# astro-turing/Integrating-diagenetic-equations-using-Python

Hardware: AMD Instinct MI355X
Metric: grid-point-steps/sec (5 fields, fp64) (higher is better)
Workload: dtype f64

## Files before the change

integrating-diagenetic-equations-using-python_amd/csrc/marl_api.hip:

```cpp
#include <hip/hip_runtime.h>

#include <dlfcn.h>

#include <cmath>
#include <cstdarg>
#include <cstdio>
#include <cstring>
#include <string>
#include <vector>

#include "../../include/marl_hip.h"
#include "marl_kernels.h"
#include "marl_rk23_ctl.h"
#include "marl_rk4_watch_ctl.h"
#include "marl_radau.h"
#include "marl_radau_cr.h"
#include "marl_radau_batch.h"
#include "marl_radau_wg.h"
#include "marl_bdf.h"
#include "marl_bdf_wg.h"
#include "marl_bdf_batch.h"
#include "marl_devbuf.h"

using namespace marl;
// ... 19 lines not shown
    size_t part_cap = 0;
    unsigned* sq = nullptr;
    size_t sq_cap = 0;
    unsigned sq_item_base = 0, sq_level_base = 0;
    bool sq_test_raise = false;
    int64_t sq_max_items = 0x7fffffff;
    unsigned* sq_sticky = nullptr;
    unsigned* sq_host = nullptr;
    bool sq_pending = false;
    int cus = 0;
    Rk45Stream* rs = nullptr;
    double* rs_grec = nullptr;
    unsigned* rs_host = nullptr;
    unsigned rs_arrive_base = 0, rs_epoch_base = 0, rs_grab_base = 0, rs_G = 0, rs_grabs_per_attempt = 0;
    int rs_occ[3][2] = {{0, 0}, {0, 0}, {0, 0}};
    int64_t rk45_stream = 1;
    int64_t dd_stream = 0;
    int64_t rk45_stream_attempts = 4096;
    double* rec = nullptr;
    Rk45Ctrl* dctrl = nullptr;
    Rk45Ctrl* hctrl = nullptr;
    double* hrec = nullptr;
    double* ddt = nullptr;
    double* hdt = nullptr;
    double* sw_teval = nullptr;
    size_t sw_teval_cap = 0;
    int64_t* sw_ndone = nullptr;
    double* sw_tev = nullptr;
    size_t sw_tev_cap = 0;
    double* dop_k = nullptr;
    size_t dop_k_cap = 0;
    double* rk4w_recs = nullptr;
    size_t rk4w_recs_cap = 0;
    int64_t dop_grid_extra = -1;
    double* dd_send = nullptr;
    double* dd_gathered = nullptr;
    double* dd_recs = nullptr;
    int dd_rank = 0, dd_world = 1;
    int64_t dd_max_attempts = 0;
    void* rccl_lib = nullptr;
    void* rccl_comm = nullptr;
    int (*rccl_allgather)(const void*, void*, size_t, int, void*, hipStream_t) = nullptr;
    int (*rccl_destroy)(void*) = nullptr;
    double* rd_arena = nullptr;
    size_t rd_cap = 0;
    double* rd_host = nullptr;
    double* zc_h = nullptr;
    double* zc_d = nullptr;
    bool zc_on = false;
    int64_t rk4_variant = -1, sweep_variant = -1, host_layout = LAYOUT_TILED, poll = 64;
    int64_t rk4_stream = 1;
    int64_t rk4_small = 1;
    int64_t rk4_chain = 1;
    int64_t rk4_stream_third = 1;
    double* stream_c = nullptr;
    size_t stream_c_cap = 0;
    int64_t implicit_zero_copy = 1;
    int64_t radau_fused_solve = 3;
    int64_t radau_solver = 0;
    int64_t radau_cr = -1;
    int64_t radau_cr_min_n = 2048;
    int64_t radau_cr_small = 3;
    int64_t radau_cr_small_min_n = 205;
    int64_t bdf_solve_wg = 1;
    int64_t radau_cr_tail = 1;
    int64_t radau_sweep_wg = 3;
    int64_t terminal[7] = {0, 0, 0, 0, 0, 0, 0};
    std::string err;
};

static bool has_terminal(const marl_ctx* ctx)
{
    for (int e = 0; e < 7; e++)
        if (ctx->terminal[e] > 0) return true;
    return false;
}

static int fail(marl_ctx* ctx, int code, const char* fmt, ...);
#define NO_TERMINAL(ctx, entry) \
    if (has_terminal(ctx)) return fail(ctx, -1, "%s: terminal monitors are not supported by this entry (marl_set_terminal)", entry);

static int fail(marl_ctx* ctx, int code, const char* fmt, ...)
{
    char msg[512];
    va_list ap;
    va_start(ap, fmt);
    vsnprintf(msg, sizeof msg, fmt, ap);
    va_end(ap);
    if (ctx) ctx->err = msg; else g_create_error = msg;
    return code;
}

#define HIP_OK(ctx, call)                                                                         \
    do {                                                                                          \
        hipError_t e_ = (call);                                                                   \
        if (e_ != hipSuccess) return fail(ctx, -100 - (int)e_, "%s failed: %s", #call, hipGetErrorString(e_)); \
    } while (0)

#define LAUNCH_OK(ctx)                                                                            \
    do {                                                                                          \
        hipError_t e_ = hipGetLastError();                                                        \
        if (e_ != hipSuccess) return fail(ctx, -100 - (int)e_, "kernel launch failed: %s", hipGetErrorString(e_)); \
    } while (0)

#ifdef MARL_LAB_CLOCK45
extern "C" int marl_lab_read_clock45(unsigned long long* dst, size_t n)
// ... 227 lines not shown
        return fail(ctx, -2, "rk4: the streamed time loop gave up waiting for a neighbouring tile (rk4_stream_kernel); the state is invalid");
    }
    return 0;
}

int marl_set_terminal(marl_ctx* ctx, const int64_t terminal[7])
{
    if (!ctx) return -1;
    for (int e = 0; terminal && e < 7; e++)
        if (terminal[e] < 0) return fail(ctx, -1, "marl_set_terminal: limit %d is negative (0: never terminal; k > 0: stop at the k-th occurrence)", e);
    for (int e = 0; e < 7; e++) ctx->terminal[e] = terminal ? terminal[e] : 0;
    return 0;
}

int marl_synchronize(marl_ctx* ctx)
{
    if (!ctx) return -1;
    HIP_OK(ctx, hipStreamSynchronize(ctx->stream));
    return stream_check(ctx);
}

int marl_set_option(marl_ctx* ctx, const char* name, int64_t value)
{
    if (!ctx || !name) return -1;
    const std::string n(name);
    if (n == "rk4_variant") ctx->rk4_variant = value;
    else if (n == "rk45_variant") { }
    else if (n == "sweep_variant") ctx->sweep_variant = value;
    else if (n == "host_layout") ctx->host_layout = value ? LAYOUT_TILED : LAYOUT_FIELD_MAJOR;
    else if (n == "poll_interval") ctx->poll = value > 0 ? value : 1;
    else if (n == "radau_solver") {
#ifdef MARL_LAB_BLOCK_THOMAS
        ctx->radau_solver = value ? 1 : 0;
#else
        if (value) return fail(ctx, -1, "marl_set_option: radau_solver = 1 (sequential block Thomas, the cross-check of the cyclic-reduction solver) is compiled into lab builds only (-DMARL_LAB_BLOCK_THOMAS)");
        ctx->radau_solver = 0;
#endif
    }
    else if (n == "radau_cr") ctx->radau_cr = (value < 0) ? -1 : std::min<int64_t>(value, radau::CR_MAX_LEVELS);
    else if (n == "radau_cr_min_n") ctx->radau_cr_min_n = std::max<int64_t>(value, 4);
    else if (n == "radau_cr_small") ctx->radau_cr_small = value < 0 ? 0 : std::min<int64_t>(value, radau::CR_WG_MAX_LEVELS);
    else if (n == "radau_cr_small_min_n") ctx->radau_cr_small_min_n = std::max<int64_t>(value, 32);
    else if (n == "radau_cr_tail") ctx->radau_cr_tail = value ? 1 : 0;
    else if (n == "bdf_solve_wg") ctx->bdf_solve_wg = value ? 1 : 0;
    else if (n == "radau_fused_solve") ctx->radau_fused_solve = value < 0 ? 0 : (value > 3 ? 3 : value);
    else if (n == "radau_sweep_wg") ctx->radau_sweep_wg = value < 0 ? 0 : (value > 3 ? 3 : value);
    else if (n == "implicit_zero_copy") ctx->implicit_zero_copy = value ? 1 : 0;
    else if (n == "rk4_stream") ctx->rk4_stream = value < 0 ? 0 : (value > 2 ? 2 : value);
    else if (n == "rk45_stream") ctx->rk45_stream = value < 0 ? 0 : (value > 2 ? 2 : value);
    else if (n == "dd_stream") ctx->dd_stream = value < 0 ? 0 : (value > 2 ? 2 : value);
    else if (n == "rk45_stream_attempts") ctx->rk45_stream_attempts = value < 1 ? 1 : std::min<int64_t>(value, 1 << 20);
    else if (n == "rk4_small") ctx->rk4_small = value ? 1 : 0;
    else if (n == "rk4_chain") ctx->rk4_chain = value < 0 ? 0 : std::min<int64_t>(value, kChainMax);
    else if (n == "rk4_stream_third") ctx->rk4_stream_third = value ? 1 : 0;
    else if (n == "rk4_stream_test_raise") ctx->sq_test_raise = value != 0;
    else if (n == "rk4_stream_max_items") ctx->sq_max_items = value > 0 ? std::min<int64_t>(value, 0x7fffffff) : 0x7fffffff;
    else if (n == "no_reuse") {
        for (auto& c : ctx->hconsts) c.hot.no_reuse = value ? 1 : 0;
        HIP_OK(ctx, hipSetDevice(ctx->device));
        HIP_OK(ctx, hipStreamSynchronize(ctx->stream));
        HIP_OK(ctx, hipMemcpy(ctx->dconsts, ctx->hconsts.data(), sizeof(DevConsts) * ctx->hconsts.size(), hipMemcpyHostToDevice));
    }
    else return fail(ctx, -1, "marl_set_option: unknown option '%s'", name);
    return 0;
}

int marl_get_constants(const marl_ctx* ctx, int64_t inst, double out[19])
{
    if (!ctx || inst < 0 || inst >= ctx->batch || !out) return -1;
    const DevConsts& d = ctx->hconsts[inst];
    const HotConsts& c = d.hot;
    const double* x = &ctx->extra[4 * inst];
    const double v[19] = {x[0], c.nu1, c.nu2, c.KRat, c.dCa, c.dCO3, c.delta, c.Da, c.lambda_, x[1], x[2], c.rhorat,
                          c.presum, x[3], c.dPhi, PECLET_MIN, PECLET_MAX, (double)d.mask_lo, (double)d.mask_hi};
    memcpy(out, v, sizeof v);
    return 0;
}

int64_t marl_state_doubles(const marl_ctx* ctx, int layout) { return ctx ? state_doubles(ctx->slab.n_buf, layout) : -1; }

}

#ifndef MARL_LAB
static inline int64_t inst_stride(const marl_ctx* ctx, int layout) { return state_doubles(ctx->slab.n_buf, layout); }

static inline unsigned blocks256(int64_t n) { return (unsigned)((n + 255) / 256); }

static const ZBatch kNoBatch{0, nullptr, 0, 0, nullptr};

static int launch_rhs_fm(marl_ctx* ctx, const double* y, double* dydt, int64_t nstates, unsigned cnt = 1, const ZBatch& zb = kNoBatch,
                         int const_stride = 0)
{
    const dim3 grid(blocks256(ctx->slab.n_buf), (unsigned)nstates, cnt);
    const int64_t stride = inst_stride(ctx, LAYOUT_FIELD_MAJOR);
    if (ctx->var_dphi)
        hipLaunchKernelGGL((rhs_kernel<LAYOUT_FIELD_MAJOR, true>), grid, dim3(256), 0, ctx->stream, y, dydt, ctx->dconsts, ctx->slab, stride, const_stride, zb);
    else
        hipLaunchKernelGGL(rhs_kernel<LAYOUT_FIELD_MAJOR>, grid, dim3(256), 0, ctx->stream, y, dydt, ctx->dconsts, ctx->slab, stride, const_stride, zb);
    LAUNCH_OK(ctx);
    return 0;
}

static int launch_rhs(marl_ctx* ctx, const double* y, double* dydt, int layout, int64_t nstates = 0)
{
    if (layout != LAYOUT_TILED) return launch_rhs_fm(ctx, y, dydt, nstates > 0 ? nstates : ctx->batch, 1, kNoBatch, nstates > 0 ? 0 : 1);
    const dim3 grid(blocks256(ctx->slab.n_buf), (unsigned)(nstates > 0 ? nstates : ctx->batch));
// ... 99 lines not shown
    return 0;
}

static int default_rk4_depth(const marl_ctx* ctx)
{
    if (ctx->var_dphi) return kVdRk4Depth;
    if (ctx->rk4_variant >= 0 && ctx->rk4_variant < kNumRk4Depths) return kRk4Depths[ctx->rk4_variant];
    const int64_t n = ctx->slab.out_hi - ctx->slab.out_lo;
    return n <= 98304 ? 16 : (n <= 262144 ? 8 : 4);
}

#ifndef MARL_LAB_STREAM_BLK
#define MARL_LAB_STREAM_BLK 256
#endif
template <int NSTEPS, bool VD = false>
static void launch_stream_t(marl_ctx* ctx, double* a, double* b, int layout, double dt, unsigned levels, unsigned tiles, unsigned blocks, double* c = nullptr)
{
    if (layout == LAYOUT_TILED)
        hipLaunchKernelGGL((rk4_stream_kernel<MARL_LAB_STREAM_BLK, LAYOUT_TILED, NSTEPS, VD>), dim3(blocks), dim3(MARL_LAB_STREAM_BLK), 0, ctx->stream, a, b, ctx->dconsts, ctx->slab, dt,
                           levels, tiles, ctx->sq, ctx->sq + 2, ctx->sq_sticky, ctx->sq_item_base, ctx->sq_level_base, c);
    else
        hipLaunchKernelGGL((rk4_stream_kernel<MARL_LAB_STREAM_BLK, LAYOUT_FIELD_MAJOR, NSTEPS, VD>), dim3(blocks), dim3(MARL_LAB_STREAM_BLK), 0, ctx->stream, a, b, ctx->dconsts, ctx->slab,
                           dt, levels, tiles, ctx->sq, ctx->sq + 2, ctx->sq_sticky, ctx->sq_item_base, ctx->sq_level_base, c);
}

struct ChainShape {
    int64_t items, bound;
    unsigned K, nsub_last;
};
static ChainShape chain_shape(int64_t n, int64_t K)
{
    constexpr int64_t H = 16, V = 256 - 2 * H, W = 256 - H;
    static_assert(V % H == 0 && W % H == 0, "a clipped chain could be narrower than the halo");
    const int64_t bound = V * ((n - 1) / V), L = V + W * (K - 1);
    const int64_t chains = (bound + L - 1) / L;
    int64_t nsub_last = 0;
    if (chains > 0) {
        const int64_t R = bound - (chains - 1) * L;
        nsub_last = R <= V ? 1 : 1 + (R - V + W - 1) / W;
    }
    return {chains + 1, bound, (unsigned)K, (unsigned)nsub_last};
}

static int64_t rk4_chain_auto(int64_t n, int64_t resident)
{
    for (int64_t K = 8; K >= 2; K--)
        if (chain_shape(n, K).items >= 2 * resident) return K;
    return 1;
}

template <int LAYOUT>
static void launch_chain_t(marl_ctx* ctx, double* a, double* b, double dt, unsigned levels, const ChainShape& sh, unsigned blocks, double* c)
{
    hipLaunchKernelGGL((rk4_chain_kernel<256, LAYOUT, 4>), dim3(blocks), dim3(256), 0, ctx->stream, a, b, ctx->dconsts, ctx->slab, dt, levels,
                       (unsigned)sh.items, ctx->sq, ctx->sq + 2, ctx->sq_sticky, ctx->sq_item_base, ctx->sq_level_base, c, sh.K, sh.nsub_last, sh.bound);
}

static int rk4_stream(marl_ctx* ctx, double* a, double* b, int layout, double dt, int per, int64_t levels, double** result)
{
    const int64_t n = ctx->slab.out_hi - ctx->slab.out_lo, V = MARL_LAB_STREAM_BLK - 8 * per;
    if (!ctx->cus) {
        hipDeviceProp_t prop;
        HIP_OK(ctx, hipGetDeviceProperties(&prop, ctx->device));
        ctx->cus = prop.multiProcessorCount;
    }
    int64_t K = 1;
    if (per == 4 && !ctx->var_dphi && MARL_LAB_STREAM_BLK == 256 && ctx->rk4_chain > 0)
        K = ctx->rk4_chain == 1 ? rk4_chain_auto(n, 4 * (int64_t)ctx->cus) : ctx->rk4_chain;
    const ChainShape shape = chain_shape(n, K);
    const int64_t tiles = K >= 2 ? shape.items : (n + V - 1) / V;
    if (!ctx->sq_host) HIP_OK(ctx, hipHostMalloc((void**)&ctx->sq_host, sizeof(unsigned), hipHostMallocDefault));
    if (!ctx->sq_sticky) {
        HIP_OK(ctx, hipMalloc((void**)&ctx->sq_sticky, sizeof(unsigned)));
        HIP_OK(ctx, hipMemsetAsync(ctx->sq_sticky, 0, sizeof(unsigned), ctx->stream));
    }
    if (ctx->sq_cap < (size_t)tiles + 2 || ctx->sq_level_base > (1u << 30)) {
        if (ctx->sq_cap < (size_t)tiles + 2) {
            if (ctx->sq) HIP_OK(ctx, hipFree(ctx->sq));
            ctx->sq = nullptr;
            ctx->sq_cap = 0;
            HIP_OK(ctx, hipMalloc((void**)&ctx->sq, ((size_t)tiles + 2) * sizeof(unsigned)));
            ctx->sq_cap = (size_t)tiles + 2;
        }
        HIP_OK(ctx, hipMemsetAsync(ctx->sq, 0, ctx->sq_cap * sizeof(unsigned), ctx->stream));
        ctx->sq_item_base = ctx->sq_level_base = 0;
    }
    if (ctx->sq_test_raise) {
        HIP_OK(ctx, hipMemsetAsync(ctx->sq_sticky, 1, sizeof(unsigned), ctx->stream));
        ctx->sq_test_raise = false;
    }
    while (levels > 0) {
        const int64_t cap = (ctx->sq_max_items / tiles) & ~(int64_t)1;
        const int64_t lv = std::min<int64_t>(levels, std::max<int64_t>(cap, 2));
        const unsigned blocks = (unsigned)std::min<int64_t>(lv * tiles, (4 * 256 / MARL_LAB_STREAM_BLK) * (int64_t)ctx->cus);
        double* c = nullptr;
        if (ctx->rk4_stream_third && levels == lv && (lv & 1) && lv >= 3) {
            const size_t need = (size_t)state_doubles(ctx->slab.n_buf, layout);
            if (ctx->stream_c_cap < need) {
                if (ctx->stream_c) HIP_OK(ctx, hipFree(ctx->stream_c));
                ctx->stream_c = nullptr; ctx->stream_c_cap = 0;
                HIP_OK(ctx, hipMalloc((void**)&ctx->stream_c, need * sizeof(double)));
                ctx->stream_c_cap = need;
            }
            c = ctx->stream_c;
        }
        if (K >= 2) {
            if (layout == LAYOUT_TILED) launch_chain_t<LAYOUT_TILED>(ctx, a, b, dt, (unsigned)lv, shape, blocks, c);
            else launch_chain_t<LAYOUT_FIELD_MAJOR>(ctx, a, b, dt, (unsigned)lv, shape, blocks, c);
// ... 3147 lines not shown
```

integrating-diagenetic-equations-using-python_amd/csrc/marl_kernels.h:

```cpp
#pragma once
#include <type_traits>

#include "marl_math.h"
#include "marl_brent.h"
#include "marl_rk_ctrl.h"
#include "marl_rk_terminal.h"

namespace marl {

enum : int { LAYOUT_FIELD_MAJOR = 0, LAYOUT_TILED = 1 };

template <int LAYOUT>
__device__ __forceinline__ int64_t at(int f, int64_t i, int64_t ld)
{
    if constexpr (LAYOUT == LAYOUT_FIELD_MAJOR)
        return (int64_t)f * ld + i;
    else
        return (i >> 6) * (int64_t)(NF * 64) + f * 64 + (i & 63);
}

struct Slab {
    int64_t n_buf;
    int64_t goff;
    int64_t ld;
    int64_t out_lo;
    int64_t out_hi;
};

__device__ __forceinline__ double nanmin(double a, double b) { return (a < b || a != a) ? a : b; }
__device__ __forceinline__ double nanmax(double a, double b) { return (a > b || a != a) ? a : b; }
template <bool FINITE = false>
__device__ __forceinline__ double mon_min(double a, double b) { return FINITE ? __builtin_fmin(a, b) : nanmin(a, b); }
template <bool FINITE = false>
__device__ __forceinline__ double mon_max(double a, double b) { return FINITE ? __builtin_fmax(a, b) : nanmax(a, b); }


#ifdef MARL_LAB_PHASE_CLOCK
__device__ unsigned long long marl_lab_phase[8];
#define MARL_PHASE_MARK(k) do { const unsigned long long t_ = __builtin_amdgcn_s_memtime(); ph_acc[k] += t_ - ph_last; ph_last = t_; } while (0)
#else
#define MARL_PHASE_MARK(k) do { } while (0)
#endif

#define MARL_ONCE _Pragma("unroll") for (int once_ = 0; once_ < 1; once_++)
#define MARL_FIELDS _Pragma("unroll") for (int f = 0; f < NF; f++)

template <int BLK, bool REUSE = true, bool VD = false, int SEAM = 0>
struct StencilBlock {
    static constexpr int EDGE_DOUBLES = 2 * NF * BLK;
    static constexpr bool CACHE_LDS = PC_LDS_SLOTS > 0;
    static constexpr bool CACHE = REUSE && (EDGE_DOUBLES + TABLE_DOUBLES + PC_LDS_SLOTS * BLK) * 8 <= 60 * 1024;
    static constexpr int CACHE_DOUBLES = CACHE ? PC_LDS_SLOTS * BLK : 0;
    static constexpr int LDS_DOUBLES = EDGE_DOUBLES + TABLE_DOUBLES + CACHE_DOUBLES;

    double* lds;
    Tables T;
    HotConsts K;
    const DevConsts* C;
    int tid;
    int parity;
    unsigned masks;
    static constexpr bool EDGE_ONCE = CACHE;
    unsigned edge_cells;
    __device__ __forceinline__ bool edge_wave() const
    {
        if constexpr (SEAM > 0) {
            unsigned e = edge_cells;
            asm volatile("" : "+s"(e));
            return e & 1u;
        } else if constexpr (EDGE_ONCE) return edge_cells & 1u;
        else return __builtin_amdgcn_ballot_w64(is_edge() != 0) != 0;
    }
    bool w_zone = false;
    __device__ __forceinline__ unsigned edge_word() const { unsigned e = edge_cells; asm volatile("" : "+s"(e)); return e; }
    __device__ __forceinline__ unsigned is_first() const { if constexpr (SEAM > 0) return (unsigned)tid + 1u == ((edge_word() >> 8) & 0x1ffu); else return masks & 1u; }
    __device__ __forceinline__ unsigned is_last() const { if constexpr (SEAM > 0) return (unsigned)tid + 1u == ((edge_word() >> 20) & 0x1ffu); else return (masks >> 8) & 1u; }
    __device__ __forceinline__ unsigned in_zone() const { if constexpr (SEAM > 0) return w_zone; else return (masks >> 16) & 1u; }
    __device__ __forceinline__ unsigned is_edge() const { return masks & 0x101u; }
    PointCache<(CACHE && CACHE_LDS) ? BLK : 0> cache;
    bool reuse_live = false;
    static constexpr int SEAM_STRIDE = 16, SEAM_READS = 0x10000, SEAM_WAVE0 = 0x20000, SEAM_WAVEW = 0x40000;
    static_assert(SEAM < BLK, "the recording lane is a lane of the window");
    double* seam = nullptr;
    int seam_pos = 0;
#ifdef MARL_LAB_PHASE_CLOCK
    unsigned long long ph_acc[6] = {0, 0, 0, 0, 0, 0}, ph_last = __builtin_amdgcn_s_memtime();
    __device__ __forceinline__ void phase_flush()
    {
        if (threadIdx.x == 0)
            for (int k = 0; k < 6; k++) atomicAdd(&marl_lab_phase[k], ph_acc[k]);
    }
#endif

    __device__ __forceinline__ StencilBlock(double* lds_, int64_t g0, const DevConsts* __restrict__ c)
        : lds(lds_), T(load_tables(lds_ + EDGE_DOUBLES, BLK)), K(load_hot(c)), C(c), tid(threadIdx.x), parity(0)
    {
        if constexpr (SEAM > 0) set_interior(false);
        else set_window(g0);
        if constexpr (CACHE && CACHE_LDS) cache.s = lds_ + EDGE_DOUBLES + TABLE_DOUBLES + tid;
    }

    __device__ __forceinline__ void rebind(int t)
    {
        tid = t;
        if constexpr (CACHE && CACHE_LDS) cache.s = lds + EDGE_DOUBLES + TABLE_DOUBLES + t;
    }

    __device__ __forceinline__ void set_window(int64_t g)
    {
        const int64_t N = C->N, mlo = C->mask_lo, mhi = C->mask_hi;
        masks = ((g == 0) ? 1u : 0u) | ((g == N - 1) ? 0x100u : 0u) | ((g >= mlo && g < mhi) ? 0x10000u : 0u);
        edge_cells = 0;
        if constexpr (EDGE_ONCE) edge_cells = (__builtin_amdgcn_ballot_w64(is_edge() != 0) != 0) ? 1u : 0u;
    }

    __device__ __forceinline__ void set_window_seam(int64_t gw)
    {
        const int64_t N = C->N, mlo = C->mask_lo, mhi = C->mask_hi;
        const int64_t g = gw + tid;
        w_zone = g >= mlo && g < mhi;
        masks = 0;
        const int wave = __builtin_amdgcn_readfirstlane(tid) >> 6;
        const int64_t t0 = -gw, t1 = N - 1 - gw;
        unsigned e = 0;
        if (t0 >= 0 && t0 < BLK) e |= (((unsigned)t0 + 1u) << 8) | ((int)(t0 >> 6) == wave ? 1u : 0u);
        if (t1 >= 0 && t1 < BLK) e |= (((unsigned)t1 + 1u) << 20) | ((int)(t1 >> 6) == wave ? 1u : 0u);
        edge_cells = __builtin_amdgcn_readfirstlane(e);
    }

    __device__ __forceinline__ void set_interior(bool zone)
    {
        w_zone = zone;
        masks = 0;
        edge_cells = 0;
    }

    template <int MODE = TR_PLAIN>
    __device__ __forceinline__ void eval(const double (&ys)[NF], double (&k)[NF], PointAux& aux)
    {
        MARL_PHASE_MARK(4);
        double* e = lds + parity * (NF * BLK);
#pragma unroll
        for (int f = 0; f < NF; f++) e[f * BLK + tid] = ys[f];
        if constexpr (SEAM > 0) {
            if (seam_pos & SEAM_WAVEW) {
                int tw = tid;
                asm volatile("" : "+v"(tw));
                if (tw == SEAM) {
                    double* rec = seam + (seam_pos & 0xffff);
#pragma unroll
                    for (int f = 0; f < NF; f++) rec[f] = ys[f];
                }
            }
        }
        MARL_PHASE_MARK(0);
        PointLocal pl;
        MARL_ONCE point_local<CACHE ? MODE : TR_PLAIN, (CACHE && CACHE_LDS) ? BLK : 0, VD>(ys, in_zone(), K, C, T, pl, aux, cache, reuse_live);
        MARL_PHASE_MARK(1);
        __syncthreads();
        MARL_PHASE_MARK(2);
        const int tl = tid > 0 ? tid - 1 : 0;
        const int tr = tid < BLK - 1 ? tid + 1 : BLK - 1;
        double left[NF], right[NF];
#pragma unroll
        for (int f = 0; f < NF; f++) left[f] = e[f * BLK + tl];
        if constexpr (SEAM > 0) {
            if ((seam_pos & (SEAM_WAVE0 | SEAM_READS)) == (SEAM_WAVE0 | SEAM_READS)) {
                int t0 = tid;
                asm volatile("" : "+v"(t0));
                if (t0 == 0) {
                    const double* prev = seam + ((seam_pos & 0xffff) ^ 8);
#pragma unroll
                    for (int f = 0; f < NF; f++) left[f] = prev[f];
                }
            }
            seam_pos += SEAM_STRIDE;
        }
        const bool need_right_solids = __builtin_amdgcn_ballot_w64(!pl.upw) != 0;
        if constexpr (CACHE) {
#pragma unroll
            for (int f = 2; f < NF; f++) right[f] = e[f * BLK + tr];
            asm volatile("" : "=v"(right[0]), "=v"(right[1]));
            if (need_right_solids) {
                right[0] = e[tr];
                right[1] = e[BLK + tr];
            }
        } else {
#pragma unroll
            for (int f = 0; f < NF; f++) right[f] = (f >= 2 || need_right_solids) ? e[f * BLK + tr] : 0.0;
        }
        parity ^= 1;
        MARL_ONCE {
            double um[NF], up[NF];
#pragma unroll
            for (int f = 0; f < NF; f++) { um[f] = left[f]; up[f] = right[f]; }
            if (edge_wave()) {
                if (is_last()) {
#pragma unroll
                    for (int f = 0; f < NF; f++) up[f] = ghost_upper(f, ys[f], um[f]);
                }
                if constexpr (SEAM > 0) {
                    size_t off = offsetof(DevConsts, bc);
                    asm volatile("" : "+s"(off));
                    const double* bcp = reinterpret_cast<const double*>(reinterpret_cast<const char*>(C) + off);
                    double bcv[NF];
#pragma unroll
                    for (int f = 0; f < NF; f++) bcv[f] = bcp[f];
                    if (is_first()) {
#pragma unroll
                        for (int f = 0; f < NF; f++) um[f] = ghost_lower(bcv[f], ys[f]);
                    }
                } else if (is_first()) {
#pragma unroll
                    for (int f = 0; f < NF; f++) um[f] = ghost_lower(C->bc[f], ys[f]);
                }
            }
            point_rates<VD, true, !CACHE>(ys, um, up, K, T, pl, k, need_right_solids);
        }
#ifdef MARL_LAB_PHASE_CLOCK
        asm volatile("" :: "v"(k[0]), "v"(k[4]));
        MARL_PHASE_MARK(3);
        ph_acc[5]++;
#endif
    }
};

template <int BLK, int NQ, int NMIN, bool FINITE = false>
__device__ __forceinline__ void block_reduce(double (&q)[NQ], double* scratch)
{
    const int lane = threadIdx.x & 63, wave = threadIdx.x >> 6;
    constexpr int NW = BLK / 64;
    auto combine = [](int j, double a, double o) { return (j == 0) ? a + o : (j <= NMIN ? mon_min<FINITE>(a, o) : mon_max<FINITE>(a, o)); };
// ... 343 lines not shown
#pragma unroll
            for (int f = 0; f < NF; f++) __hip_atomic_store(dst + at<LAYOUT>(f, l, S.ld), y[f], __ATOMIC_RELAXED, __HIP_MEMORY_SCOPE_AGENT);
        }
        __atomic_signal_fence(__ATOMIC_SEQ_CST);
        __builtin_amdgcn_s_waitcnt(0);
        __atomic_signal_fence(__ATOMIC_SEQ_CST);
        __syncthreads();
        if (threadIdx.x == 0) {
            __hip_atomic_store(&done[tile], level_base + level + 1u, __ATOMIC_RELAXED, __HIP_MEMORY_SCOPE_AGENT);
#ifdef MARL_LAB_BROKEN_STREAM_LATCH
            s_item = __hip_atomic_fetch_add(&queue[0], 1u, __ATOMIC_RELAXED, __HIP_MEMORY_SCOPE_AGENT) - item_base;
            s_abort = 0;
#endif
        }
    }
}

struct ChainArgs {
    double *bufA, *bufB;
    const DevConsts* consts;
    Slab S;
    double dt;
    unsigned levels, items;
    unsigned *queue, *done, *sticky;
    unsigned item_base, level_base;
    double* bufC;
    unsigned K, nsub_last;
    int64_t bound;
};
static_assert(offsetof(ChainArgs, S) == 24 && offsetof(ChainArgs, dt) == 64 && offsetof(ChainArgs, queue) == 80 && offsetof(ChainArgs, bufC) == 112 &&
              offsetof(ChainArgs, bound) == 128 && sizeof(ChainArgs) == 136, "the argument list of rk4_chain_kernel, in order");
typedef const __attribute__((address_space(4))) ChainArgs* ChainArgsPtr;
__device__ __forceinline__ ChainArgsPtr chain_args()
{
    ChainArgsPtr a = (ChainArgsPtr)__builtin_amdgcn_kernarg_segment_ptr();
    asm volatile("" : "+s"(a));
    return a;
}

template <int BLK, int LAYOUT, int NSTEPS>
__global__ void __launch_bounds__(BLK) __attribute__((amdgpu_waves_per_eu(4, 8)))
rk4_chain_kernel(double* bufA, double* bufB, const DevConsts* __restrict__ consts, Slab S, double dt, unsigned levels, unsigned items,
                 unsigned* queue, unsigned* done, unsigned* sticky, unsigned item_base, unsigned level_base, double* bufC,
                 unsigned K, unsigned nsub_last, int64_t bound)
{
    constexpr int H = 4 * NSTEPS;
    constexpr int V = BLK - 2 * H;
    constexpr int W = BLK - H;
    static_assert(V > 0, "window too small for the fused halo");
    using SB = StencilBlock<BLK, true, false, BLK - H - 1>;
    __shared__ double lds[SB::LDS_DOUBLES];
    __shared__ double seam[H * SB::SEAM_STRIDE];
    __shared__ unsigned s_item, s_abort;
    const DevConsts& C = consts[0];
    SB sb(lds, 0, consts);
    sb.seam = seam;
    dt = pin_uniform(dt);
    const unsigned total = levels * items;
    const unsigned chains = items - 1;

    while (true) {
        __syncthreads();
        typedef __attribute__((address_space(1))) unsigned* GlobalWords;
        ChainArgsPtr G = chain_args();
        unsigned *const queue = (unsigned*)(GlobalWords)G->queue, *const done = (unsigned*)(GlobalWords)G->done,
                 *const sticky = (unsigned*)(GlobalWords)G->sticky;
        const unsigned items = G->items, item_base = G->item_base, level_base = G->level_base;
        if (threadIdx.x == 0) {
            s_item = __hip_atomic_fetch_add(&queue[0], 1u, __ATOMIC_RELAXED, __HIP_MEMORY_SCOPE_AGENT) - item_base;
            s_abort = 0;
        }
        __syncthreads();
        const unsigned item = __builtin_amdgcn_readfirstlane(s_item);
        if (item >= total) break;
        const unsigned level = item / items, tile = item - level * items;
        if (level > 0) {
            if (threadIdx.x < 3) {
                const int64_t t = (int64_t)tile - 1 + threadIdx.x;
                if (t >= 0 && t < (int64_t)items) {
                    unsigned spins = 0;
                    while ((int)(__hip_atomic_load(&done[t], __ATOMIC_RELAXED, __HIP_MEMORY_SCOPE_AGENT) - (level_base + level)) < 0) {
                        __builtin_amdgcn_s_sleep(4);
                        if (++spins > STREAM_SPIN_LIMIT ||
                            ((spins & 255u) == 0 && __hip_atomic_load(sticky, __ATOMIC_RELAXED, __HIP_MEMORY_SCOPE_AGENT))) {
                            __hip_atomic_store(sticky, 1u, __ATOMIC_RELAXED, __HIP_MEMORY_SCOPE_AGENT);
                            s_abort = 1;
                            break;
                        }
                    }
                }
            }
            __syncthreads();
            if (s_abort) break;
        }
        const double* src;
        double* dst;
        unsigned nsub;
        int64_t first, clip;
        {
            ChainArgsPtr A = chain_args();
            double *const pA = A->bufA, *const pB = A->bufB, *const pC = A->bufC;
            const unsigned nlev = A->levels, KK = A->K, nlast = A->nsub_last;
            const int64_t olo = A->S.out_lo, ohi = A->S.out_hi, bnd = A->bound;
            src = (const double*)(const __attribute__((address_space(1))) double*)(pC ? (level == 0 ? pA : ((level & 1u) ? pB : pC)) : ((level & 1u) ? pB : pA));
            dst = (double*)(__attribute__((address_space(1))) double*)(pC ? (level + 1 == nlev ? pA : ((level & 1u) ? pC : pB)) : ((level & 1u) ? pA : pB));
            const bool chain = tile < chains;
// ... 1539 lines not shown
```

integrating-diagenetic-equations-using-python_amd/csrc/marl_math.h:

```cpp
#pragma once
#include <hip/hip_runtime.h>
#include <stddef.h>
#include <stdint.h>

#include "marl_tables.h"

namespace marl {

constexpr int NF = 5;

struct HotConsts {
    double inv_dx, inv_dx2;
    double presum, rhorat;
    double KRat, nu1, nu2;
    double lambda_, Da, delta;
    double dCa, dCO3, dPhi;
    double pe_cCa, pe_cCO3, pe_Phi;
    double m1, m2, n1, n2;
    double hdx;
    double pe_smax;
    double Dal;
    double Da_nu1, Dal_nu2;
    double rr10;
    double dPhi_dx2;
// ... 98 lines not shown
__device__ __forceinline__ double pow_sat(double b, double e, const Tables& T)
{
    const double r = fast_exp(e * fast_log(b, T), T);
    return (b == 0.0) ? 0.0 : r;
}

template <bool SERIES>
__device__ __forceinline__ double fv_sigma(double Pe, double W, const Tables& T)
{
    const double a = fabs(Pe);
    double s = 0.0;
    if (a > PECLET_MAX) {
        s = (W > 0.0) ? 1.0 : ((W < 0.0) ? -1.0 : W);
    } else if (!(a < PECLET_MIN)) {
        if (SERIES && a <= FV_SERIES_MAX) {
            const double x2 = Pe * Pe;
            double p = 2.3106432599002624e-11;
            p = __builtin_fma(p, x2, -2.2805151204592183e-10);
            p = __builtin_fma(p, x2, 2.2507846516808994e-09);
            p = __builtin_fma(p, x2, -2.2214608789979678e-08);
            p = __builtin_fma(p, x2, 2.1925947851873778e-07);
            p = __builtin_fma(p, x2, -2.1644042808063972e-06);
            p = __builtin_fma(p, x2, 2.1377799155576935e-05);
            p = __builtin_fma(p, x2, -1.0 / 4725);
            p = __builtin_fma(p, x2, 2.0 / 945);
            p = __builtin_fma(p, x2, -1.0 / 45);
            p = __builtin_fma(p, x2, 1.0 / 3);
            s = p * Pe;
        } else {
            s = (1.0 + 2.0 * rcp_nr(fast_exp(2.0 * Pe, T) - 1.0)) - rcp_nr(Pe);
        }
    }
    return s;
}

__device__ __forceinline__ double ghost_lower(double bc, double u0) { return 2.0 * bc - u0; }
__device__ __forceinline__ double ghost_upper(int f, double uN1, double uN2) { return (f < 2) ? 2.0 * uN1 - uN2 : uN1; }

struct PointAux {
    double U, W;
};

enum : int { TR_PLAIN = 0, TR_FILL = 1, TR_REUSE = 2, TR_AUTO = 3 };
constexpr double REUSE_LIMIT = 5e-5;
constexpr double REUSE_TINY = 2e-6;

#ifndef MARL_CACHE_LDS_SLOTS
#define MARL_CACHE_LDS_SLOTS 4
#endif
enum : int { PC_INVPHI, PC_INVOM, PC_INVDEN, PC_IB, PC_E, PC_TC, PC_SLOTS };
constexpr int PC_FIRST_LDS = PC_SLOTS - (MARL_CACHE_LDS_SLOTS < PC_SLOTS ? MARL_CACHE_LDS_SLOTS : PC_SLOTS);
constexpr int PC_LDS_SLOTS = PC_SLOTS - PC_FIRST_LDS;

template <int STRIDE>
struct PointCache {
    static constexpr int FIRST_LDS = STRIDE > 0 ? PC_FIRST_LDS : PC_SLOTS;
    double Phi, O2, cPhi, nib;
    double* s;
    double v[FIRST_LDS > 0 ? FIRST_LDS : 1];
    bool fv_quiet;
    __device__ __forceinline__ double get(int j) const { return j < FIRST_LDS ? v[j] : s[(j - FIRST_LDS) * STRIDE]; }
    __device__ __forceinline__ void set(int j, double x) { if (j < FIRST_LDS) v[j] = x; else s[(j - FIRST_LDS) * STRIDE] = x; }
};

template <int MODE>
__device__ __forceinline__ double ten_operand()
{
    if constexpr (MODE == TR_PLAIN) return 10.0;
    else return pin_uniform(10.0);
}

struct PointLocal {
    double Ux, R0, R1;
    double W, invPhi, G2, G3;
    double h1x, h2f;
    double Q4, DaR;
    double Wd;
    bool upw, fv_active;
    bool fv_solutes;
};

#pragma clang diagnostic push
#pragma clang diagnostic ignored "-Wsometimes-uninitialized"
template <int MODE, int STRIDE, bool VD = false, bool LEGACY = false>
__device__ __forceinline__ void point_local(const double (&uc)[NF], bool in_mask, const HotConsts& K, const DevConsts* __restrict__ C,
                                            const Tables& T, PointLocal& pl, PointAux& aux, PointCache<STRIDE>& pc, bool& live)
{
    static_assert(!LEGACY || MODE == TR_PLAIN, "the legacy operation order is the stand-alone RHS's (no transcendental cache)");
#ifdef MARL_ABLATE_CORE
    aux.U = aux.W = 0.0;
    return;
#endif
    const double CA = uc[0], CC = uc[1], c = uc[2], o = uc[3], Phi = uc[4];
    const double omPhi = 1.0 - Phi;
    const double O2 = c * o;

    double den, invPhi, invom, invden, ex, tC, tA;
    bool fv_check = K.fv != 0;
    bool reuse = false;
    if constexpr (MODE == TR_FILL) live = false;
    if ((MODE == TR_REUSE || MODE == TR_AUTO) && live) {
        const double d = Phi - pc.Phi, dO = O2 - pc.O2;
        const double v = dO * pc.nib;
        const double big = __builtin_fma(fabs(d), pc.cPhi, fabs(v));
        reuse = __builtin_amdgcn_ballot_w64(!(big < REUSE_LIMIT)) == 0;
        live = reuse;
        if (reuse) {
            const bool tiny = __builtin_amdgcn_ballot_w64(!(big < REUSE_TINY)) == 0;
            const double invPhi0 = pc.get(PC_INVPHI), invom0 = pc.get(PC_INVOM), invden0 = pc.get(PC_INVDEN), ib0 = pc.get(PC_IB);
            const double e0 = pc.get(PC_E), tC0 = pc.get(PC_TC);
            const double x = d * invPhi0, y = d * invom0, u = dO * ib0;
            double l1p, ip, w, gy;
            double da;
            if (__builtin_expect(tiny, 1)) {
                l1p = x * __builtin_fma(x, -0.5, 1.0);
                const double t10 = invPhi0 * __builtin_fma(-x, x, x);
                ip = invPhi0 - t10;
                da = 10.0 * t10;
                w = v * __builtin_fma(u, -0.5, 1.0);
                gy = __builtin_fma(y, 1.0 + y, 1.0);
            } else {
                l1p = x * __builtin_fma(x, __builtin_fma(x, 1.0 / 3, -0.5), 1.0);
                ip = invPhi0 * __builtin_fma(-x, __builtin_fma(-x, 1.0 - x, 1.0), 1.0);
                da = -10.0 * (ip - invPhi0);
                w = v * __builtin_fma(u, __builtin_fma(u, 1.0 / 3, -0.5), 1.0);
                gy = __builtin_fma(y, __builtin_fma(y, 1.0 + y, 1.0), 1.0);
            }
            const double z = -2.0 * l1p * invden0;
            invPhi = ip;
            invom = invom0 * gy;
            if (__builtin_expect(tiny, 1)) {
                invden = __builtin_fma(-invden0, __builtin_fma(-z, z, z), invden0);
                ex = e0 * __builtin_fma(da, __builtin_fma(da, 0.5, 1.0), 1.0);
                tC = tC0 * __builtin_fma(w, __builtin_fma(w, 0.5, 1.0), 1.0);
            } else {
                invden = invden0 * __builtin_fma(-z, __builtin_fma(-z, 1.0 - z, 1.0), 1.0);
                ex = e0 * __builtin_fma(da, __builtin_fma(da, __builtin_fma(da, 1.0 / 6, 0.5), 1.0), 1.0);
                tC = tC0 * __builtin_fma(w, __builtin_fma(w, __builtin_fma(w, 1.0 / 6, 0.5), 1.0), 1.0);
            }
            fv_check = !pc.fv_quiet;
            if (fv_check) {
                asm volatile("");
                den = rcp_nr(invden);
            }
        }
    }
    if (!reuse) {
#ifdef MARL_ABLATE_LOG
        const double L = Phi - 1.0;
#else
        const double L = fast_log(Phi, T);
#endif
        den = __builtin_fma(-2.0, L, 1.0);
        const double pd = Phi * den, od = omPhi * den, po = Phi * omPhi;
#ifdef MARL_ABLATE_RCP
        const double rall = 2.0 - pd * omPhi;
#else
        const double rall = rcp_nr(pd * omPhi);
#endif
        invPhi = rall * od, invom = rall * pd, invden = rall * po;
#ifdef MARL_ABLATE_EXP
        ex = 0.01 * __builtin_fma(-10.0, invPhi, 10.0);
#else
        const double ten = ten_operand<MODE>();
        ex = fast_exp(__builtin_fma(-ten, invPhi, ten), T);
#endif
        const bool over = O2 > 1.0;
        const double nsel = over ? K.n1 : K.n2;
#ifdef MARL_ABLATE_POW
        const double pwC = fabs(O2 - 1.0) * nsel;
#else
        const double pwC = pow_sat(fabs(O2 - 1.0), nsel, T);
#endif
        tC = (LEGACY ? (over ? 1.0 : -K.nu2) : (over ? K.Dal : -K.Dal_nu2)) * pwC;
        if (K.generic_p0) {
            asm volatile("");
            const double y1 = C->p0_n1, y2 = C->p0_n2, nu2 = C->hot.nu2;
            const double pcw = (O2 == 1.0) ? (over ? y1 : y2) : pwC;
            tC = (LEGACY ? 1.0 : K.Dal) * (over ? pcw - nu2 * y2 : y1 - nu2 * pcw);
        }
        if constexpr (MODE == TR_FILL || MODE == TR_AUTO) {
            const double ib = (K.generic_p0 | K.no_reuse) ? __builtin_nan("") : rcp_nr(O2 - 1.0);
            pc.Phi = Phi; pc.O2 = O2; pc.nib = nsel * ib;
            pc.cPhi = fmax(fmax(fabs(invPhi), fabs(invom)), fmax(12.0 * (invPhi * invPhi), 2.2 * fabs(invPhi * invden)));
            pc.set(PC_INVPHI, invPhi); pc.set(PC_INVOM, invom); pc.set(PC_INVDEN, invden); pc.set(PC_E, ex);
            pc.set(PC_IB, ib); pc.set(PC_TC, tC);
            live = true;
        }
    }
    {
        const double O3 = O2 * K.KRat;
        const bool under = O3 < 1.0;
        tA = O3 - O3;
        if (!under || in_mask) {
#ifdef MARL_ABLATE_POWA
            const double pwA = fabs(O3 - 1.0) * (under ? K.m2 : K.m1);
#else
            const double pwA = pow_sat(fabs(O3 - 1.0), under ? K.m2 : K.m1, T);
#endif
            tA = (LEGACY ? (under ? 1.0 : -K.nu1) : (under ? K.Da : -K.Da_nu1)) * pwA;
        }
        if (K.generic_p0) {
            asm volatile("");
            const double z1 = C->p0_m1, z2 = C->p0_m2, nu1 = C->hot.nu1;
            const double mask = in_mask ? 1.0 : 0.0;
            const double pa = (O3 == 1.0) ? (under ? z2 : z1) : ((!under || in_mask) ? fast_exp((under ? K.m2 : K.m1) * fast_log(fabs(O3 - 1.0), T), T) : 0.0);
            tA = (LEGACY ? 1.0 : K.Da) * (under ? pa * mask - nu1 * z1 : z2 * mask - nu1 * pa);
        }
    }
    const double rF = LEGACY ? K.rhorat * (1.0 - ex) : __builtin_fma(-K.rhorat, ex, K.rhorat);
    const double t2 = rF * (Phi * Phi);
    const double W = K.presum - t2;
    const double U = __builtin_fma(t2 * Phi, invom, K.presum);
    aux.U = U;
    aux.W = W;
    double wpe = fabs(W) * K.pe_Phi;
    if constexpr (VD) {
        const double dPhi = K.auxcon * ((1.0 - ex) * (Phi * Phi)) * (Phi * invom);
        wpe = fabs(W) * (K.pe_Phi * (K.dPhi * rcp_nr(dPhi)));
    }

    const double DA = LEGACY ? K.Da * (CA * tA) : CA * tA;
    const double DC = LEGACY ? K.Dal * (CC * tC) : CC * tC;
    const double DmD = DA - DC;
    const double DaR = omPhi * DmD;
    pl.upw = U > 0.0;
    pl.Ux = fabs(U * K.inv_dx);
    pl.R0 = __builtin_fma(CA, DmD, -DA);
    pl.R1 = __builtin_fma(CC, DmD, DC);

    bool fv_active = false;
    if constexpr (MODE == TR_PLAIN) pl.Wd = 0.0;
#ifdef MARL_ABLATE_FV
    fv_check = false;
#endif
    pl.fv_solutes = MODE != TR_PLAIN;
    if (fv_check) {
        asm volatile("");
        const double Wd = W * den;
// ... 111 lines not shown
```

Measured before the change: 53.66 billion.

## Add RK4 exchange kernel with cell-major LDS stencil and paired cache slots

Adds an rk4_exchange_kernel variant of the chained RK4 streaming kernel, selected by default through a new rk4_exchange option. It stores the neighbour-exchange stencil in LDS cell-major with a padded pitch, so each point's fields are written and read with 16-byte vector accesses. It also packs the transcendental cache slots in pairs so they move as double2 loads and stores. The aim is fewer LDS instructions per stencil evaluation. The kernel also asserts an LDS budget that allows four workgroups per CU. The cost is padding and possible bank conflicts from the strided cell layout.

Result: faster. 54.51 billion (median of 6 runs) (+1.6%).

```diff
diff --git a/integrating-diagenetic-equations-using-python_amd/csrc/marl_api.hip b/integrating-diagenetic-equations-using-python_amd/csrc/marl_api.hip
--- a/integrating-diagenetic-equations-using-python_amd/csrc/marl_api.hip
+++ b/integrating-diagenetic-equations-using-python_amd/csrc/marl_api.hip
@@ -95,6 +95,7 @@
     int64_t rk4_stream = 1;
     int64_t rk4_small = 1;
     int64_t rk4_chain = 1;
+    int64_t rk4_exchange = 1;
     int64_t rk4_stream_third = 1;
     double* stream_c = nullptr;
     size_t stream_c_cap = 0;
@@ -428,6 +429,11 @@
     else if (n == "rk45_stream_attempts") ctx->rk45_stream_attempts = value < 1 ? 1 : std::min<int64_t>(value, 1 << 20);
     else if (n == "rk4_small") ctx->rk4_small = value ? 1 : 0;
     else if (n == "rk4_chain") ctx->rk4_chain = value < 0 ? 0 : std::min<int64_t>(value, kChainMax);
+#ifdef MARL_LAB_XCH_PARTS
+    else if (n == "rk4_exchange") ctx->rk4_exchange = value < 0 ? 0 : std::min<int64_t>(value, 3);
+#else
+    else if (n == "rk4_exchange") ctx->rk4_exchange = value ? 1 : 0;
+#endif
     else if (n == "rk4_stream_third") ctx->rk4_stream_third = value ? 1 : 0;
     else if (n == "rk4_stream_test_raise") ctx->sq_test_raise = value != 0;
     else if (n == "rk4_stream_max_items") ctx->sq_max_items = value > 0 ? std::min<int64_t>(value, 0x7fffffff) : 0x7fffffff;
@@ -633,8 +639,18 @@
 template <int LAYOUT>
 static void launch_chain_t(marl_ctx* ctx, double* a, double* b, double dt, unsigned levels, const ChainShape& sh, unsigned blocks, double* c)
 {
-    hipLaunchKernelGGL((rk4_chain_kernel<256, LAYOUT, 4>), dim3(blocks), dim3(256), 0, ctx->stream, a, b, ctx->dconsts, ctx->slab, dt, levels,
-                       (unsigned)sh.items, ctx->sq, ctx->sq + 2, ctx->sq_sticky, ctx->sq_item_base, ctx->sq_level_base, c, sh.K, sh.nsub_last, sh.bound);
+#define MARL_CHAIN_LAUNCH(KERNEL)                                                                                                                \
+    hipLaunchKernelGGL(KERNEL, dim3(blocks), dim3(256), 0, ctx->stream, a, b, ctx->dconsts, ctx->slab, dt, levels, (unsigned)sh.items, ctx->sq, \
+                       ctx->sq + 2, ctx->sq_sticky, ctx->sq_item_base, ctx->sq_level_base, c, sh.K, sh.nsub_last, sh.bound)
+    switch (ctx->rk4_exchange) {
+        case 0: MARL_CHAIN_LAUNCH((rk4_chain_kernel<256, LAYOUT, 4>)); break;
+#ifdef MARL_LAB_XCH_PARTS
+        case 1: MARL_CHAIN_LAUNCH((rk4_exchange_kernel<256, LAYOUT, 4, XCH_CELL>)); break;
+        case 2: MARL_CHAIN_LAUNCH((rk4_exchange_kernel<256, LAYOUT, 4, XCH_PAIRS>)); break;
+#endif
+        default: MARL_CHAIN_LAUNCH((rk4_exchange_kernel<256, LAYOUT, 4>)); break;
+    }
+#undef MARL_CHAIN_LAUNCH
 }
 
 static int rk4_stream(marl_ctx* ctx, double* a, double* b, int layout, double dt, int per, int64_t levels, double** result)
diff --git a/integrating-diagenetic-equations-using-python_amd/csrc/marl_kernels.h b/integrating-diagenetic-equations-using-python_amd/csrc/marl_kernels.h
--- a/integrating-diagenetic-equations-using-python_amd/csrc/marl_kernels.h
+++ b/integrating-diagenetic-equations-using-python_amd/csrc/marl_kernels.h
@@ -45,9 +45,12 @@
 #define MARL_ONCE _Pragma("unroll") for (int once_ = 0; once_ < 1; once_++)
 #define MARL_FIELDS _Pragma("unroll") for (int f = 0; f < NF; f++)
 
-template <int BLK, bool REUSE = true, bool VD = false, int SEAM = 0>
+enum : int { XCH_CELL = 1, XCH_PAIRS = 2 };
+template <int BLK, bool REUSE = true, bool VD = false, int SEAM = 0, int XCH = 0>
 struct StencilBlock {
-    static constexpr int EDGE_DOUBLES = 2 * NF * BLK;
+    static constexpr bool CELL = (XCH & XCH_CELL) != 0, PAIRS = (XCH & XCH_PAIRS) != 0;
+    static constexpr int PITCH = NF + 1;
+    static constexpr int EDGE_DOUBLES = 2 * (CELL ? PITCH : NF) * BLK;
     static constexpr bool CACHE_LDS = PC_LDS_SLOTS > 0;
     static constexpr bool CACHE = REUSE && (EDGE_DOUBLES + TABLE_DOUBLES + PC_LDS_SLOTS * BLK) * 8 <= 60 * 1024;
     static constexpr int CACHE_DOUBLES = CACHE ? PC_LDS_SLOTS * BLK : 0;
@@ -77,7 +80,9 @@
     __device__ __forceinline__ unsigned is_last() const { if constexpr (SEAM > 0) return (unsigned)tid + 1u == ((edge_word() >> 20) & 0x1ffu); else return (masks >> 8) & 1u; }
     __device__ __forceinline__ unsigned in_zone() const { if constexpr (SEAM > 0) return w_zone; else return (masks >> 16) & 1u; }
     __device__ __forceinline__ unsigned is_edge() const { return masks & 0x101u; }
-    PointCache<(CACHE && CACHE_LDS) ? BLK : 0> cache;
+    static_assert(XCH == 0 || (CACHE && PC_LDS_SLOTS == 4 && (EDGE_DOUBLES + TABLE_DOUBLES) % 2 == 0), "XCH: 16-byte accesses, two pairs of cache slots");
+    PointCache<(CACHE && CACHE_LDS) ? BLK : 0, PAIRS> cache;
+    __device__ __forceinline__ double* cache_slots(double* l, int t) const { return l + EDGE_DOUBLES + TABLE_DOUBLES + (PAIRS ? 2 * t : t); }
     bool reuse_live = false;
     static constexpr int SEAM_STRIDE = 16, SEAM_READS = 0x10000, SEAM_WAVE0 = 0x20000, SEAM_WAVEW = 0x40000;
     static_assert(SEAM < BLK, "the recording lane is a lane of the window");
@@ -97,13 +102,13 @@
     {
         if constexpr (SEAM > 0) set_interior(false);
         else set_window(g0);
-        if constexpr (CACHE && CACHE_LDS) cache.s = lds_ + EDGE_DOUBLES + TABLE_DOUBLES + tid;
+        if constexpr (CACHE && CACHE_LDS) cache.s = cache_slots(lds_, tid);
     }
 
     __device__ __forceinline__ void rebind(int t)
     {
         tid = t;
-        if constexpr (CACHE && CACHE_LDS) cache.s = lds + EDGE_DOUBLES + TABLE_DOUBLES + t;
+        if constexpr (CACHE && CACHE_LDS) cache.s = cache_slots(lds, t);
     }
 
     __device__ __forceinline__ void set_window(int64_t g)
@@ -139,9 +144,16 @@
     __device__ __forceinline__ void eval(const double (&ys)[NF], double (&k)[NF], PointAux& aux)
     {
         MARL_PHASE_MARK(4);
-        double* e = lds + parity * (NF * BLK);
-#pragma unroll
-        for (int f = 0; f < NF; f++) e[f * BLK + tid] = ys[f];
+        double* e = lds + parity * ((CELL ? PITCH : NF) * BLK);
+        if constexpr (CELL) {
+            double* own = e + PITCH * tid;
+            reinterpret_cast<double2v*>(own)[0] = double2v{ys[0], ys[1]};
+            reinterpret_cast<double2v*>(own)[1] = double2v{ys[2], ys[3]};
+            own[4] = ys[4];
+        } else {
+#pragma unroll
+            for (int f = 0; f < NF; f++) e[f * BLK + tid] = ys[f];
+        }
         if constexpr (SEAM > 0) {
             if (seam_pos & SEAM_WAVEW) {
                 int tw = tid;
@@ -162,8 +174,15 @@
         const int tl = tid > 0 ? tid - 1 : 0;
         const int tr = tid < BLK - 1 ? tid + 1 : BLK - 1;
         double left[NF], right[NF];
-#pragma unroll
-        for (int f = 0; f < NF; f++) left[f] = e[f * BLK + tl];
+        if constexpr (CELL) {
+            const double* lc = e + PITCH * tl;
+            const double2v s01 = reinterpret_cast<const double2v*>(lc)[0], s23 = reinterpret_cast<const double2v*>(lc)[1];
+            left[0] = s01.x; left[1] = s01.y; left[2] = s23.x; left[3] = s23.y;
+            left[4] = lc[4];
+        } else {
+#pragma unroll
+            for (int f = 0; f < NF; f++) left[f] = e[f * BLK + tl];
+        }
         if constexpr (SEAM > 0) {
             if ((seam_pos & (SEAM_WAVE0 | SEAM_READS)) == (SEAM_WAVE0 | SEAM_READS)) {
                 int t0 = tid;
@@ -177,7 +196,17 @@
             seam_pos += SEAM_STRIDE;
         }
         const bool need_right_solids = __builtin_amdgcn_ballot_w64(!pl.upw) != 0;
-        if constexpr (CACHE) {
+        if constexpr (CELL) {
+            const double* rc = e + PITCH * tr;
+            const double2v s23 = reinterpret_cast<const double2v*>(rc)[1];
+            right[2] = s23.x; right[3] = s23.y;
+            right[4] = rc[4];
+            asm volatile("" : "=v"(right[0]), "=v"(right[1]));
+            if (need_right_solids) {
+                const double2v s01 = reinterpret_cast<const double2v*>(rc)[0];
+                right[0] = s01.x; right[1] = s01.y;
+            }
+        } else if constexpr (CACHE) {
 #pragma unroll
             for (int f = 2; f < NF; f++) right[f] = e[f * BLK + tr];
             asm volatile("" : "=v"(right[0]), "=v"(right[1]));
@@ -627,6 +656,144 @@
     __shared__ double lds[SB::LDS_DOUBLES];
     __shared__ double seam[H * SB::SEAM_STRIDE];
     __shared__ unsigned s_item, s_abort;
+    const DevConsts& C = consts[0];
+    SB sb(lds, 0, consts);
+    sb.seam = seam;
+    dt = pin_uniform(dt);
+    const unsigned total = levels * items;
+    const unsigned chains = items - 1;
+
+    while (true) {
+        __syncthreads();
+        typedef __attribute__((address_space(1))) unsigned* GlobalWords;
+        ChainArgsPtr G = chain_args();
+        unsigned *const queue = (unsigned*)(GlobalWords)G->queue, *const done = (unsigned*)(GlobalWords)G->done,
+                 *const sticky = (unsigned*)(GlobalWords)G->sticky;
+        const unsigned items = G->items, item_base = G->item_base, level_base = G->level_base;
+        if (threadIdx.x == 0) {
+            s_item = __hip_atomic_fetch_add(&queue[0], 1u, __ATOMIC_RELAXED, __HIP_MEMORY_SCOPE_AGENT) - item_base;
+            s_abort = 0;
+        }
+        __syncthreads();
+        const unsigned item = __builtin_amdgcn_readfirstlane(s_item);
+        if (item >= total) break;
+        const unsigned level = item / items, tile = item - level * items;
+        if (level > 0) {
+            if (threadIdx.x < 3) {
+                const int64_t t = (int64_t)tile - 1 + threadIdx.x;
+                if (t >= 0 && t < (int64_t)items) {
+                    unsigned spins = 0;
+                    while ((int)(__hip_atomic_load(&done[t], __ATOMIC_RELAXED, __HIP_MEMORY_SCOPE_AGENT) - (level_base + level)) < 0) {
+                        __builtin_amdgcn_s_sleep(4);
+                        if (++spins > STREAM_SPIN_LIMIT ||
+                            ((spins & 255u) == 0 && __hip_atomic_load(sticky, __ATOMIC_RELAXED, __HIP_MEMORY_SCOPE_AGENT))) {
+                            __hip_atomic_store(sticky, 1u, __ATOMIC_RELAXED, __HIP_MEMORY_SCOPE_AGENT);
+                            s_abort = 1;
+                            break;
+                        }
+                    }
+                }
+            }
+            __syncthreads();
+            if (s_abort) break;
+        }
+        const double* src;
+        double* dst;
+        unsigned nsub;
+        int64_t first, clip;
+        {
+            ChainArgsPtr A = chain_args();
+            double *const pA = A->bufA, *const pB = A->bufB, *const pC = A->bufC;
+            const unsigned nlev = A->levels, KK = A->K, nlast = A->nsub_last;
+            const int64_t olo = A->S.out_lo, ohi = A->S.out_hi, bnd = A->bound;
+            src = (const double*)(const __attribute__((address_space(1))) double*)(pC ? (level == 0 ? pA : ((level & 1u) ? pB : pC)) : ((level & 1u) ? pB : pA));
+            dst = (double*)(__attribute__((address_space(1))) double*)(pC ? (level + 1 == nlev ? pA : ((level & 1u) ? pC : pB)) : ((level & 1u) ? pA : pB));
+            const bool chain = tile < chains;
+            nsub = chain ? (tile + 1 == chains ? nlast : KK) : 1u;
+            first = olo - H + (chain ? (int64_t)tile * (V + (int64_t)W * (KK - 1)) : bnd);
+            clip = chain ? olo + bnd : ohi;
+        }
+#pragma unroll 1
+        for (unsigned j = 0; j < nsub; j++) {
+            int tid = threadIdx.x;
+            asm volatile("" : "+v"(tid));
+            sb.rebind(tid);
+            ChainArgsPtr A = chain_args();
+            const int64_t n_buf = A->S.n_buf, goff = A->S.goff, ld = A->S.ld;
+            const int64_t lw = first + (int64_t)j * W, gw = lw + goff;
+            const int64_t mlo = C.mask_lo, mhi = C.mask_hi;
+            auto neg = [](int64_t a, int64_t b) {
+                int32_t hi = (int32_t)(((uint64_t)a - (uint64_t)b) >> 32);
+                asm("" : "+s"(hi));
+                return hi;
+            };
+            const int32_t out_any = neg(lw, 0) | neg(n_buf, lw + BLK) | neg(gw, 1) | neg(C.N - 1, gw + BLK);
+            const int32_t zone_part = neg(gw, mlo) | neg(mhi, gw + BLK);
+            const int32_t zone_some = neg(mlo, gw + BLK) & neg(gw, mhi);
+            const bool interior = out_any >= 0 && (zone_part >= 0 || zone_some >= 0);
+            const int64_t l = lw + tid;
+            bool in = true;
+            int64_t la = l;
+            if (!interior) {
+                asm volatile("");
+                in = l >= 0 && l < n_buf;
+                la = in ? l : 0;
+            }
+            double y[NF];
+#pragma unroll
+            for (int f = 0; f < NF; f++) y[f] = __hip_atomic_load(src + at<LAYOUT>(f, la, ld), __ATOMIC_RELAXED, __HIP_MEMORY_SCOPE_AGENT);
+            if (interior) {
+                sb.set_interior(zone_part >= 0);
+            } else {
+                asm volatile("");
+#pragma unroll
+                for (int f = 0; f < NF; f++) y[f] = in ? y[f] : C.bc[f];
+                sb.set_window_seam(gw);
+            }
+            sb.reuse_live = false;
+            const int wave = __builtin_amdgcn_readfirstlane(tid) >> 6;
+            sb.seam_pos = (int)(j & 1u) * 8 + (j ? SB::SEAM_READS : 0) + (wave == 0 ? SB::SEAM_WAVE0 : 0)
+                          + (wave == (BLK - H - 1) / 64 ? SB::SEAM_WAVEW : 0);
+            const int64_t room = clip - lw;
+            int hi = neg(room, BLK - H) < 0 ? (int)room : BLK - H;
+            asm volatile("" : "+s"(hi));
+            rk4_advance<NSTEPS>(sb, y, dt);
+            int sp = sb.seam_pos;
+            asm volatile("" : "+s"(sp));
+            const int lo = (sp & SB::SEAM_READS) ? 0 : H;
+            int ts = threadIdx.x;
+            asm volatile("" : "+v"(ts));
+            const int64_t ls = first + (int64_t)j * W + ts;
+            if (ts >= lo && ts < hi) {
+                int64_t lds_ = 0;
+                if constexpr (LAYOUT == LAYOUT_FIELD_MAJOR) lds_ = chain_args()->S.ld;
+#pragma unroll
+                for (int f = 0; f < NF; f++) __hip_atomic_store(dst + at<LAYOUT>(f, ls, lds_), y[f], __ATOMIC_RELAXED, __HIP_MEMORY_SCOPE_AGENT);
+            }
+        }
+        __atomic_signal_fence(__ATOMIC_SEQ_CST);
+        __builtin_amdgcn_s_waitcnt(0);
+        __atomic_signal_fence(__ATOMIC_SEQ_CST);
+        __syncthreads();
+        if (threadIdx.x == 0) __hip_atomic_store(&done[tile], level_base + level + 1u, __ATOMIC_RELAXED, __HIP_MEMORY_SCOPE_AGENT);
+    }
+}
+
+template <int BLK, int LAYOUT, int NSTEPS, int XCH = XCH_CELL | XCH_PAIRS>
+__global__ void __launch_bounds__(BLK) __attribute__((amdgpu_waves_per_eu(4, 8)))
+rk4_exchange_kernel(double* bufA, double* bufB, const DevConsts* __restrict__ consts, Slab S, double dt, unsigned levels, unsigned items,
+                    unsigned* queue, unsigned* done, unsigned* sticky, unsigned item_base, unsigned level_base, double* bufC,
+                    unsigned K, unsigned nsub_last, int64_t bound)
+{
+    constexpr int H = 4 * NSTEPS;
+    constexpr int V = BLK - 2 * H;
+    constexpr int W = BLK - H;
+    static_assert(V > 0, "window too small for the fused halo");
+    using SB = StencilBlock<BLK, true, false, BLK - H - 1, XCH>;
+    __shared__ __attribute__((aligned(16))) double lds[SB::LDS_DOUBLES];
+    __shared__ double seam[H * SB::SEAM_STRIDE];
+    __shared__ unsigned s_item, s_abort;
+    static_assert((SB::LDS_DOUBLES + H * SB::SEAM_STRIDE) * 8 + 8 <= 40960, "four workgroups per CU: 160 KB of LDS");
     const DevConsts& C = consts[0];
     SB sb(lds, 0, consts);
     sb.seam = seam;
diff --git a/integrating-diagenetic-equations-using-python_amd/csrc/marl_math.h b/integrating-diagenetic-equations-using-python_amd/csrc/marl_math.h
--- a/integrating-diagenetic-equations-using-python_amd/csrc/marl_math.h
+++ b/integrating-diagenetic-equations-using-python_amd/csrc/marl_math.h
@@ -174,15 +174,35 @@
 constexpr int PC_FIRST_LDS = PC_SLOTS - (MARL_CACHE_LDS_SLOTS < PC_SLOTS ? MARL_CACHE_LDS_SLOTS : PC_SLOTS);
 constexpr int PC_LDS_SLOTS = PC_SLOTS - PC_FIRST_LDS;
 
-template <int STRIDE>
+typedef double double2v __attribute__((ext_vector_type(2)));
+
+template <int STRIDE, bool PAIRS = false>
 struct PointCache {
     static constexpr int FIRST_LDS = STRIDE > 0 ? PC_FIRST_LDS : PC_SLOTS;
+    static_assert(!PAIRS || (STRIDE > 0 && PC_LDS_SLOTS == 4), "two pairs of LDS slots");
     double Phi, O2, cPhi, nib;
     double* s;
     double v[FIRST_LDS > 0 ? FIRST_LDS : 1];
     bool fv_quiet;
-    __device__ __forceinline__ double get(int j) const { return j < FIRST_LDS ? v[j] : s[(j - FIRST_LDS) * STRIDE]; }
-    __device__ __forceinline__ void set(int j, double x) { if (j < FIRST_LDS) v[j] = x; else s[(j - FIRST_LDS) * STRIDE] = x; }
+    __device__ __forceinline__ double get(int j) const
+    {
+        if constexpr (PAIRS) {
+            if (j >= FIRST_LDS) return reinterpret_cast<const double2v*>(s + ((j - FIRST_LDS) / 2) * 2 * STRIDE)[0][(j - FIRST_LDS) % 2];
+        }
+        return j < FIRST_LDS ? v[j] : s[(j - FIRST_LDS) * STRIDE];
+    }
+    __device__ __forceinline__ void set(int j, double x)
+    {
+        if constexpr (PAIRS) {
+            if (j >= FIRST_LDS) { s[((j - FIRST_LDS) / 2) * 2 * STRIDE + (j - FIRST_LDS) % 2] = x; return; }
+        }
+        if (j < FIRST_LDS) v[j] = x; else s[(j - FIRST_LDS) * STRIDE] = x;
+    }
+    __device__ __forceinline__ void set_pair(int j, double x0, double x1)
+    {
+        static_assert(PAIRS, "set_pair: the paired layout only");
+        reinterpret_cast<double2v*>(s + ((j - FIRST_LDS) / 2) * 2 * STRIDE)[0] = double2v{x0, x1};
+    }
 };
 
 template <int MODE>
@@ -204,9 +224,9 @@
 
 #pragma clang diagnostic push
 #pragma clang diagnostic ignored "-Wsometimes-uninitialized"
-template <int MODE, int STRIDE, bool VD = false, bool LEGACY = false>
+template <int MODE, int STRIDE, bool VD = false, bool LEGACY = false, bool PAIRS = false>
 __device__ __forceinline__ void point_local(const double (&uc)[NF], bool in_mask, const HotConsts& K, const DevConsts* __restrict__ C,
-                                            const Tables& T, PointLocal& pl, PointAux& aux, PointCache<STRIDE>& pc, bool& live)
+                                            const Tables& T, PointLocal& pl, PointAux& aux, PointCache<STRIDE, PAIRS>& pc, bool& live)
 {
     static_assert(!LEGACY || MODE == TR_PLAIN, "the legacy operation order is the stand-alone RHS's (no transcendental cache)");
 #ifdef MARL_ABLATE_CORE
@@ -305,8 +325,13 @@
             const double ib = (K.generic_p0 | K.no_reuse) ? __builtin_nan("") : rcp_nr(O2 - 1.0);
             pc.Phi = Phi; pc.O2 = O2; pc.nib = nsel * ib;
             pc.cPhi = fmax(fmax(fabs(invPhi), fabs(invom)), fmax(12.0 * (invPhi * invPhi), 2.2 * fabs(invPhi * invden)));
-            pc.set(PC_INVPHI, invPhi); pc.set(PC_INVOM, invom); pc.set(PC_INVDEN, invden); pc.set(PC_E, ex);
-            pc.set(PC_IB, ib); pc.set(PC_TC, tC);
+            if constexpr (PAIRS) {
+                pc.set(PC_INVPHI, invPhi); pc.set(PC_INVOM, invom);
+                pc.set_pair(PC_INVDEN, invden, ib); pc.set_pair(PC_E, ex, tC);
+            } else {
+                pc.set(PC_INVPHI, invPhi); pc.set(PC_INVOM, invom); pc.set(PC_INVDEN, invden); pc.set(PC_E, ex);
+                pc.set(PC_IB, ib); pc.set(PC_TC, tC);
+            }
             live = true;
         }
     }
```
